# elfi-dev/elfi

Hardware: NVIDIA H100
Metric: accepted particles/sec (higher is better)
Workload: dtype f64

## Files before the change

elfi_b200/csrc/common.cuh:

```cuda
#pragma once

#include <cuda.h>
#include <cuda_runtime.h>

#include <cstdarg>
#include <cstdint>
#include <cstdio>
#include <cstring>
#include <type_traits>

#include "../../include/elfi_b200.h"

namespace elfi {

void set_error(const char* fmt, ...);

#define ELFI_CUDA_OK(expr)                                                              \
    do {                                                                                \
        cudaError_t _e = (expr);                                                        \
        if (_e != cudaSuccess) {                                                        \
            ::elfi::set_error("%s failed: %s (%s:%d)", #expr, cudaGetErrorString(_e),   \
                              __FILE__, __LINE__);                                      \
            cudaGetLastError();       \
            return ELFI_B200_ERR_CUDA;                                                  \
        }                                                                               \
    } while (0)

#define ELFI_REQUIRE(cond, ...)                                                         \
    do {                                                                                \
        if (!(cond)) {                                                                  \
            ::elfi::set_error(__VA_ARGS__);                                             \
            return ELFI_B200_ERR_ARG;                                                   \
        }                                                                               \
    } while (0)

typedef CUresult (*tensor_map_encode_fn)(CUtensorMap*, CUtensorMapDataType, cuuint32_t, void*,
                                         const cuuint64_t*, const cuuint64_t*,
                                         const cuuint32_t*, const cuuint32_t*,
                                         CUtensorMapInterleave, CUtensorMapSwizzle,
                                         CUtensorMapL2promotion, CUtensorMapFloatOOBfill);

}

struct elfi_b200_ctx {
    int device;
    int sm_count;
    size_t smem_optin;
    elfi::tensor_map_encode_fn encode_tiled;
    void* scratch;
    size_t scratch_bytes;
    void* pinned;
    size_t pinned_bytes;
    void* dev_stage;
    size_t dev_stage_bytes;
    cudaStream_t copy_stream[2];
    cudaEvent_t copy_event[4];
};

namespace elfi {

void* ctx_scratch(elfi_b200_ctx* ctx, size_t bytes);

int make_rowmajor_f64_map(elfi_b200_ctx* ctx, const double* base, int64_t rows, int64_t cols,
                          int64_t ld, int box_rows, CUtensorMap* out);

inline bool tma_compatible(const void* base, int64_t ld) {
    return (reinterpret_cast<uintptr_t>(base) % 16 == 0) && ((ld * 8) % 16 == 0);
}

template <class Body>
int run_on_device(elfi_b200_ctx* ctx, void* stream, Body&& body) {
    ELFI_CUDA_OK(cudaSetDevice(ctx->device));
    const int rc = body(static_cast<cudaStream_t>(stream));
    if (rc != ELFI_B200_OK) return rc;
    ELFI_CUDA_OK(cudaGetLastError());
    return ELFI_B200_OK;
}

template <int LO, int HI, class F>
auto with_pow2(int k, F&& f) {
    if constexpr (LO == HI) {
        return f(std::integral_constant<int, LO>{});
    } else {
// ... 72 lines not shown
```

elfi_b200/csrc/ctx.cu:

```cuda
#include "common.cuh"

namespace elfi {

static thread_local char g_error[512] = "";

void set_error(const char* fmt, ...) {
    va_list ap;
    va_start(ap, fmt);
    vsnprintf(g_error, sizeof(g_error), fmt, ap);
    va_end(ap);
}

void* ctx_scratch(elfi_b200_ctx* ctx, size_t bytes) {
    if (bytes <= ctx->scratch_bytes) return ctx->scratch;
    size_t want = bytes + (bytes >> 2) + (1u << 20);
    want = (want + 255) & ~size_t(255);
    if (ctx->scratch) {
        if (cudaDeviceSynchronize() != cudaSuccess || cudaFree(ctx->scratch) != cudaSuccess) {
            set_error("scratch release failed: %s", cudaGetErrorString(cudaGetLastError()));
            ctx->scratch = nullptr;
            ctx->scratch_bytes = 0;
            return nullptr;
        }
        ctx->scratch = nullptr;
// ... 40 lines not shown

const char* elfi_b200_last_error(void) { return elfi::g_error; }

int elfi_b200_ctx_create(int device, elfi_b200_ctx** out) {
    ELFI_REQUIRE(out != nullptr, "ctx_create: out is NULL");
    *out = nullptr;
    int count = 0;
    ELFI_CUDA_OK(cudaGetDeviceCount(&count));
    ELFI_REQUIRE(device >= 0 && device < count, "ctx_create: device %d out of range (%d visible)",
                 device, count);
    ELFI_CUDA_OK(cudaSetDevice(device));
    cudaDeviceProp prop;
    ELFI_CUDA_OK(cudaGetDeviceProperties(&prop, device));
    if (prop.major != 9 || prop.minor != 0) {
        elfi::set_error("ctx_create: device %d is sm_%d%d; this library is built for sm_90a only",
                        device, prop.major, prop.minor);
        return ELFI_B200_ERR_UNSUPPORTED;
    }
    elfi_b200_ctx* ctx = new elfi_b200_ctx();
    memset(ctx, 0, sizeof(*ctx));
    ctx->device = device;
    ctx->sm_count = prop.multiProcessorCount;
    ctx->smem_optin = prop.sharedMemPerBlockOptin;
    void* fn = nullptr;
    cudaDriverEntryPointQueryResult qres;
    cudaError_t e = cudaGetDriverEntryPoint("cuTensorMapEncodeTiled", &fn, cudaEnableDefault, &qres);
    if (e != cudaSuccess || qres != cudaDriverEntryPointSuccess || fn == nullptr) {
        elfi::set_error("ctx_create: cuTensorMapEncodeTiled not available from the driver");
        delete ctx;
        cudaGetLastError();
        return ELFI_B200_ERR_CUDA;
    }
    ctx->encode_tiled = reinterpret_cast<elfi::tensor_map_encode_fn>(fn);
    for (int i = 0; i < 2; ++i)
        ELFI_CUDA_OK(cudaStreamCreateWithFlags(&ctx->copy_stream[i], cudaStreamNonBlocking));
    for (int i = 0; i < 4; ++i)
        ELFI_CUDA_OK(cudaEventCreateWithFlags(&ctx->copy_event[i], cudaEventDisableTiming));
    *out = ctx;
    return ELFI_B200_OK;
}

int elfi_b200_ctx_destroy(elfi_b200_ctx* ctx) {
    if (!ctx) return ELFI_B200_OK;
    cudaSetDevice(ctx->device);
    cudaDeviceSynchronize();
    if (ctx->scratch) cudaFree(ctx->scratch);
    if (ctx->dev_stage) cudaFree(ctx->dev_stage);
    if (ctx->pinned) cudaFreeHost(ctx->pinned);
    for (int i = 0; i < 2; ++i)
        if (ctx->copy_stream[i]) cudaStreamDestroy(ctx->copy_stream[i]);
    for (int i = 0; i < 4; ++i)
        if (ctx->copy_event[i]) cudaEventDestroy(ctx->copy_event[i]);
    delete ctx;
    return ELFI_B200_OK;
}

int elfi_b200_ctx_sm_count(const elfi_b200_ctx* ctx) { return ctx ? ctx->sm_count : 0; }

int elfi_b200_allgather_particles(elfi_b200_ctx* const* ctxs, int64_t n_ctx, const double* const* send,
                                  int64_t rows, int64_t width, double* const* recv,
                                  void* const* streams) {
    ELFI_REQUIRE(ctxs && send && recv && streams && n_ctx >= 1 && n_ctx <= 64,
                 "allgather_particles: bad argument");
    ELFI_REQUIRE(rows >= 0 && width >= 1, "allgather_particles: bad shape");
    for (int64_t g = 0; g < n_ctx; ++g)
        ELFI_REQUIRE(ctxs[g] && (rows == 0 || (send[g] && recv[g])), "allgather_particles: NULL entry %lld",
                     (long long)g);
    if (rows == 0) return ELFI_B200_OK;
    const size_t bytes = size_t(rows) * size_t(width) * 8;
    int caller_device = 0;
    ELFI_CUDA_OK(cudaGetDevice(&caller_device));
    struct Restore {
        int d;
        ~Restore() { cudaSetDevice(d); }
    } restore{caller_device};
    for (int64_t d = 0; d < n_ctx; ++d) {
        ELFI_CUDA_OK(cudaSetDevice(ctxs[d]->device));
        for (int64_t s = 0; s < n_ctx; ++s) {
            if (ctxs[s]->device == ctxs[d]->device) continue;
            int can = 0;
// ... 34 lines not shown
```

elfi_b200/csrc/distance.cu:

```cuda
#include <cstdlib>

#include "metric.cuh"
#include "rowstream.cuh"

namespace elfi {

struct DistParams {
    const double* obs;
    const double* W;
    double* d_out;
    uint32_t* mask;
    int K;
    int has_thr;
    const double* shift_src;
    double* mom_partial;
    const double* thr_dev;
    double thr[ELFI_B200_MAX_NESTED];
    __device__ __forceinline__ double threshold(int k) const {
        return thr_dev ? __ldg(thr_dev + k) : thr[k];
    }
};

__device__ __forceinline__ void dist_setup_shared(uint8_t* aux, const DistParams& p, int D,
                                                  bool weighted) {
    const int Dp = rs_padded_cols(D);
    double* obs_s = reinterpret_cast<double*>(aux);
    for (int j = threadIdx.x; j < Dp; j += blockDim.x) obs_s[j] = j < D ? p.obs[j] : 0.0;
    if (weighted) {
        double* w_s = obs_s + Dp;
        for (int k = 0; k < p.K; ++k)
            for (int j = threadIdx.x; j < Dp; j += blockDim.x)
                w_s[size_t(k) * Dp + j] = j < D ? p.W[size_t(k) * D + j] : 0.0;
    }
}
// ... 265 lines not shown
            rc = rowstream_launch<NestedMomentsConsumer<KMAX>>(ctx, S, ldS, B, D, aux, p, stream);
    } else {
        rc = rowstream_launch<NestedMomentsConsumer<KMAX>>(ctx, S, ldS, B, D, aux, p, stream);
    }
    if (rc) return rc;
    colmoments_flush_kernel<<<unsigned((D + 31) / 32), dim3(32, 32), 0, stream>>>(
        S, p.mom_partial, nwarps, B, D, moments);
    ELFI_CUDA_OK(cudaGetLastError());
    return ELFI_B200_OK;
}

__global__ void __launch_bounds__(256)
dist_direct_kernel(const double* __restrict__ S, int64_t ld, int64_t B, int D, DistParams p) {
    const int64_t row = int64_t(blockIdx.x) * blockDim.x + threadIdx.x;
    dist_record<false, 0>(p, p.K, row, B, threadIdx.x & 31, [&](int k) {
        const double* r = S + row * ld;
        double acc = 0.0;
        if (p.W != nullptr) {
            const double* w = p.W + size_t(k) * D;
            for (int j = 0; j < D; ++j) {
                const double d = __dsub_rn(__ldg(r + j), __ldg(p.obs + j));
                acc = __dadd_rn(acc, __dmul_rn(__ldg(w + j), __dmul_rn(d, d)));
            }
        } else {
            for (int j = 0; j < D; ++j) {
                const double d = __dsub_rn(__ldg(r + j), __ldg(p.obs + j));
                acc = __dadd_rn(acc, __dmul_rn(d, d));
            }
        }
        return sqrt(acc);
    });
}

__global__ void __launch_bounds__(1024)
compact_mask_kernel(const uint32_t* __restrict__ mask, int64_t nwords, int64_t B,
                    int32_t* __restrict__ idx, int64_t* __restrict__ n_out) {
    __shared__ int64_t warp_sums[32];
    __shared__ int64_t base_s;
    const int tid = threadIdx.x;
    const int lane = tid & 31;
    const int wid = tid >> 5;
    const int64_t first = int64_t(blockIdx.x) * 1024;

    int64_t before = 0;
    for (int64_t w = tid; w < first; w += 1024) before += __popc(mask[w]);
    for (int o = 16; o > 0; o >>= 1) before += __shfl_xor_sync(0xffffffffu, before, o);
    if (lane == 0) warp_sums[wid] = before;
    __syncthreads();
    if (tid == 0) {
        int64_t t = 0;
        for (int i = 0; i < 32; ++i) t += warp_sums[i];
        base_s = t;
    }
    __syncthreads();
    const int64_t base = base_s;
    __syncthreads();

    const int64_t w = first + tid;
    const uint32_t bits = w < nwords ? mask[w] : 0u;
    const int cnt = __popc(bits);
    int incl = cnt;
    for (int o = 1; o < 32; o <<= 1) {
        const int t = __shfl_up_sync(0xffffffffu, incl, o);
        if (lane >= o) incl += t;
    }
    if (lane == 31) warp_sums[wid] = incl;
    __syncthreads();
    if (wid == 0) {
        int64_t v = warp_sums[lane];
        int64_t inc2 = v;
        for (int o = 1; o < 32; o <<= 1) {
            const int64_t t = __shfl_up_sync(0xffffffffu, inc2, o);
            if (lane >= o) inc2 += t;
        }
        warp_sums[lane] = inc2 - v;
        if (lane == 31 && blockIdx.x == gridDim.x - 1 && n_out != nullptr) *n_out = base + inc2;
    }
    __syncthreads();
    int64_t pos = base + warp_sums[wid] + (incl - cnt);
    if (idx != nullptr) {
        uint32_t b = bits;
        while (b) {
            const int bit = __ffs(b) - 1;
            b &= b - 1;
            idx[pos++] = int32_t(w * 32 + bit);
        }
    }
}

int launch_compact_mask(const uint32_t* mask, int64_t B, int32_t* idx, int64_t* n_out,
                        cudaStream_t stream) {
    const int64_t nwords = (B + 31) / 32;
    if (nwords == 0) {
        if (n_out) ELFI_CUDA_OK(cudaMemsetAsync(n_out, 0, sizeof(int64_t), stream));
        return ELFI_B200_OK;
    }
    const unsigned blocks = unsigned((nwords + 1023) / 1024);
    compact_mask_kernel<<<blocks, 1024, 0, stream>>>(mask, nwords, B, idx, n_out);
    ELFI_CUDA_OK(cudaGetLastError());
    return ELFI_B200_OK;
}

static DistParams dist_params(const double* obs, const double* W, int64_t K,
                              const double* thr_host, const double* thr_dev, double* d_out,
                              uint32_t* mask) {
    DistParams p = {};
    p.obs = obs;
    p.W = W;
    p.d_out = d_out;
    p.mask = mask;
    p.K = int(K);
    p.has_thr = thr_host != nullptr || thr_dev != nullptr;
    p.thr_dev = thr_dev;
    if (thr_host)
        for (int k = 0; k < K; ++k) p.thr[k] = thr_host[k];
    return p;
}

int launch_dist(elfi_b200_ctx* ctx, const double* S, int64_t ldS, int64_t B, int64_t D,
                const DistParams& p, cudaStream_t stream) {
    if (B == 0) return ELFI_B200_OK;
    const double* W = p.W;
    const int K = p.K;
    const size_t aux = size_t(rs_padded_cols(D)) * 8 * (W ? (1 + K) : 1);
    if (rs_streams(ctx, S, ldS, D, aux)) {
        if (W == nullptr) return rowstream_launch<EuclidConsumer>(ctx, S, ldS, B, D, aux, p, stream);
        if (K == 1) return rowstream_launch<WeightedConsumer>(ctx, S, ldS, B, D, aux, p, stream);
        if (K <= 2) return rowstream_launch<NestedConsumer<2>>(ctx, S, ldS, B, D, aux, p, stream);
        if (K <= 3) return rowstream_launch<NestedConsumer<3>>(ctx, S, ldS, B, D, aux, p, stream);
        if (K <= 4) return rowstream_launch<NestedConsumer<4>>(ctx, S, ldS, B, D, aux, p, stream);
        if (K <= 5) return rowstream_launch<NestedConsumer<5>>(ctx, S, ldS, B, D, aux, p, stream);
// ... 182 lines not shown
    ELFI_REQUIRE(B >= 0 && D >= 1, "dist: bad shape B=%lld D=%lld", (long long)B, (long long)D);
    ELFI_REQUIRE(B == 0 || S != nullptr, "dist: S is NULL");
    ELFI_REQUIRE(obs != nullptr, "dist: obs is NULL");
    ELFI_REQUIRE(ldS >= D, "dist: ldS (%lld) < D (%lld)", (long long)ldS, (long long)D);
    ELFI_REQUIRE(K >= 1 && K <= ELFI_B200_MAX_NESTED, "dist: K=%lld outside [1, %d]",
                 (long long)K, ELFI_B200_MAX_NESTED);
    ELFI_REQUIRE(W != nullptr || K == 1, "dist: K=%lld needs a weight matrix", (long long)K);
    ELFI_REQUIRE(acc_idx == nullptr || thr != nullptr, "dist: acc_idx requires thresholds");
    ELFI_REQUIRE(B < (int64_t(1) << 31), "dist: B must fit int32 row indices");
    return ELFI_B200_OK;
}

template <class Launch>
static int dist_call(const char* who, elfi_b200_ctx* ctx, const double* S, int64_t ldS, int64_t B,
                     int64_t D, const double* obs, const double* W, int64_t K,
                     const double* thr_host, const double* thr_dev, double* d_out,
                     int32_t* acc_idx, int64_t* n_acc, void* stream_, Launch launch) {
    const double* thr = thr_host ? thr_host : thr_dev;
    int rc = check_dist_args(S, ldS, B, D, obs, W, K, thr, acc_idx);
    if (rc) return rc;
    ELFI_REQUIRE(B == 0 || d_out != nullptr, "%s: d_out is NULL", who);
    cudaStream_t stream = static_cast<cudaStream_t>(stream_);
    ELFI_CUDA_OK(cudaSetDevice(ctx->device));
    uint32_t* mask = nullptr;
    if (thr != nullptr) {
        mask = static_cast<uint32_t*>(ctx_scratch(ctx, size_t((B + 31) / 32) * 4 + 256));
        if (!mask) return ELFI_B200_ERR_NOMEM;
    }
    rc = launch(dist_params(obs, W, K, thr_host, thr_dev, d_out, mask), stream);
    if (rc) return rc;
    if (thr != nullptr && (acc_idx != nullptr || n_acc != nullptr))
        return launch_compact_mask(mask, B, acc_idx, n_acc, stream);
    return ELFI_B200_OK;
}

}

extern "C" {

int elfi_b200_dist_euclid_thr_f64(elfi_b200_ctx* ctx, const double* S, int64_t ldS, int64_t B,
                                  int64_t D, const double* obs, const double* W, int64_t K,
                                  const double* thr_host, double* d_out, int32_t* acc_idx,
                                  int64_t* n_acc, void* stream_) {
    using namespace elfi;
    ELFI_REQUIRE(ctx != nullptr, "dist: ctx is NULL");
    return dist_call("dist", ctx, S, ldS, B, D, obs, W, K, thr_host, nullptr, d_out, acc_idx, n_acc,
                     stream_, [&](const DistParams& p, cudaStream_t stream) {
                         return launch_dist(ctx, S, ldS, B, D, p, stream);
                     });
}

int elfi_b200_dist_euclid_thr_dev_f64(elfi_b200_ctx* ctx, const double* S, int64_t ldS, int64_t B,
                                      int64_t D, const double* obs, const double* W, int64_t K,
                                      const double* thr_dev, double* d_out, int32_t* acc_idx,
                                      int64_t* n_acc, void* stream_) {
    using namespace elfi;
    ELFI_REQUIRE(ctx != nullptr && thr_dev != nullptr, "dist: ctx or thr_dev is NULL");
    return dist_call("dist", ctx, S, ldS, B, D, obs, W, K, nullptr, thr_dev, d_out, acc_idx, n_acc,
                     stream_, [&](const DistParams& p, cudaStream_t stream) {
                         return launch_dist(ctx, S, ldS, B, D, p, stream);
                     });
}

int elfi_b200_dist_euclid_mom_f64(elfi_b200_ctx* ctx, const double* S, int64_t ldS, int64_t B,
                                  int64_t D, const double* obs, const double* W, int64_t K,
                                  const double* thr_host, const double* thr_dev, double* d_out,
// ... 162 lines not shown
```

elfi_b200/csrc/select.cu:

```cuda
#include <cstdlib>

#include "bitonic.cuh"
#include "eqweight.h"
#include "pairwise.cuh"

namespace elfi {

constexpr int SORT_CHUNK = 1024;
constexpr int SORT_WARPS = 8;

__global__ void __launch_bounds__(256)
sort_prepare_kernel(const double* __restrict__ keys, int64_t n, uint64_t* __restrict__ ukeys,
                    int32_t* __restrict__ vals, uint32_t* __restrict__ ghist) {
    __shared__ uint32_t h[8 * 256];
    for (int i = threadIdx.x; i < 8 * 256; i += blockDim.x) h[i] = 0;
    __syncthreads();
    const int64_t stride = int64_t(gridDim.x) * blockDim.x;
    for (int64_t i = int64_t(blockIdx.x) * blockDim.x + threadIdx.x; i < n; i += stride) {
        const uint64_t u = key_to_u64(keys[i]);
        ukeys[i] = u;
        vals[i] = int32_t(i);
#pragma unroll
        for (int p = 0; p < 8; ++p) atomicAdd(&h[p * 256 + ((u >> (8 * p)) & 255)], 1u);
    }
    __syncthreads();
    for (int i = threadIdx.x; i < 8 * 256; i += blockDim.x)
        if (h[i]) atomicAdd(&ghist[i], h[i]);
}

__device__ __forceinline__ bool pass_trivial(const uint32_t* ghist, int pass, int64_t n,
                                             uint64_t first_key) {
    return ghist[pass * 256 + ((first_key >> (8 * pass)) & 255)] == uint32_t(n);
}

__global__ void __launch_bounds__(SORT_WARPS * 32)
// ... 142 lines not shown
    const unsigned wblocks = unsigned((s.nw + SORT_WARPS - 1) / SORT_WARPS);
    int cur = 0;
    for (int pass = 0; pass < 8; ++pass) {
        sort_upsweep_kernel<<<wblocks, SORT_WARPS * 32, 0, stream>>>(s.k[cur], n, pass, s.nw, s.ghist, s.whist);
        sort_scan_kernel<<<256, 1024, 0, stream>>>(s.k[cur], n, pass, s.nw, s.ghist, s.whist);
        sort_scatter_kernel<<<wblocks, SORT_WARPS * 32, 0, stream>>>(
            s.k[cur], s.v[cur], n, pass, s.nw, s.ghist, s.whist, s.k[cur ^ 1], s.v[cur ^ 1]);
        cur ^= 1;
    }
    ELFI_CUDA_OK(cudaGetLastError());
    return ELFI_B200_OK;
}

__global__ void __launch_bounds__(256)
gather_rows_kernel(const double* __restrict__ src, int64_t ld_src, const int32_t* __restrict__ idx,
                   int64_t n, int64_t width, double* __restrict__ dst, int64_t ld_dst) {
    const int64_t total = n * width;
    const int64_t stride = int64_t(gridDim.x) * blockDim.x;
    for (int64_t t = int64_t(blockIdx.x) * blockDim.x + threadIdx.x; t < total; t += stride) {
        const int64_t i = t / width, j = t - i * width;
        dst[i * ld_dst + j] = src[int64_t(idx[i]) * ld_src + j];
    }
}

constexpr int APPEND_MAX_SRC = 8;
struct AppendSources {
    const double* ptr[APPEND_MAX_SRC];
    int64_t ld[APPEND_MAX_SRC];
    int32_t width[APPEND_MAX_SRC];
    int32_t col0[APPEND_MAX_SRC];
    int32_t n_src, total_width;
};

__global__ void __launch_bounds__(256)
accept_append_kernel(const int32_t* __restrict__ acc_idx, const int64_t* __restrict__ n_acc,
                     AppendSources src, double* __restrict__ dst, int64_t ld_dst, int64_t capacity,
                     const int64_t* __restrict__ count) {
    const int64_t base = *count;
    int64_t room = capacity - base;
    if (room < 0) room = 0;
    const int64_t rows = *n_acc < room ? *n_acc : room;
    const int64_t total = rows * src.total_width;
    const int64_t stride = int64_t(gridDim.x) * blockDim.x;
    for (int64_t t = int64_t(blockIdx.x) * blockDim.x + threadIdx.x; t < total; t += stride) {
        const int64_t j = t / src.total_width;
        const int c = int(t - j * src.total_width);
        const int64_t row = acc_idx ? int64_t(acc_idx[j]) : j;
        int k = 0;
#pragma unroll
        for (int q = 1; q < APPEND_MAX_SRC; ++q)
            if (q < src.n_src && c >= src.col0[q]) k = q;
        dst[(base + j) * ld_dst + c] = src.ptr[k][row * src.ld[k] + (c - src.col0[k])];
    }
}

__global__ void accept_count_kernel(const int64_t* __restrict__ n_acc, int64_t capacity,
                                    int64_t* __restrict__ count, int64_t* __restrict__ dropped) {
    int64_t room = capacity - *count;
    if (room < 0) room = 0;
    const int64_t rows = *n_acc < room ? *n_acc : room;
    if (dropped) *dropped += *n_acc - rows;
    *count += rows;
}

__global__ void __launch_bounds__(256)
gather2_rows_kernel(const double* __restrict__ A, int64_t ldA, int64_t nA,
                    const double* __restrict__ Bm, int64_t ldB, const int32_t* __restrict__ mapB,
                    const int32_t* __restrict__ perm, int64_t n, int64_t width,
                    double* __restrict__ dst, int64_t ld_dst) {
    const int64_t total = n * width;
    const int64_t stride = int64_t(gridDim.x) * blockDim.x;
    for (int64_t t = int64_t(blockIdx.x) * blockDim.x + threadIdx.x; t < total; t += stride) {
        const int64_t i = t / width, j = t - i * width;
        const int64_t r = perm ? perm[i] : i;
        double v;
        if (r < nA) {
            v = A[r * ldA + j];
        } else {
            const int64_t rb = mapB ? int64_t(mapB[r - nA]) : (r - nA);
            v = Bm[rb * ldB + j];
        }
        dst[i * ld_dst + j] = v;
    }
}

__global__ void __launch_bounds__(256)
merge_keys_kernel(const double* __restrict__ keysA, int64_t ldA, int64_t nA,
                  const double* __restrict__ keysB, int64_t ldB, const int32_t* __restrict__ mapB,
                  int64_t nB, double* __restrict__ out) {
    const int64_t stride = int64_t(gridDim.x) * blockDim.x;
    for (int64_t i = int64_t(blockIdx.x) * blockDim.x + threadIdx.x; i < nA + nB; i += stride) {
        if (i < nA) {
            out[i] = keysA[i * ldA];
        } else {
            const int64_t rb = mapB ? int64_t(mapB[i - nA]) : (i - nA);
// ... 296 lines not shown
        double incl = v;
        for (int o = 1; o < 32; o <<= 1) {
            const double t = __shfl_up_sync(0xffffffffu, incl, o);
            if (lane >= o) incl += t;
        }
        if (lane == 31) ws[wid] = incl;
        __syncthreads();
        double woff = 0.0;
        for (int q = 0; q < wid; ++q) woff += ws[q];
        const double carry = carry_s;
        const double c = (carry + woff + incl) / total;
        if (i < n - 1) {
            l0 += (c < alpha - eps) ? 1 : 0;
            l1 += (c < alpha + eps) ? 1 : 0;
        }
        __syncthreads();
        if (tid == 1023) carry_s = carry + woff + incl;
        __syncthreads();
    }
    for (int o = 16; o > 0; o >>= 1) {
        l0 += __shfl_xor_sync(0xffffffffu, l0, o);
        l1 += __shfl_xor_sync(0xffffffffu, l1, o);
    }
    if (lane == 0) { atomicAdd(&c0_s, l0); atomicAdd(&c1_s, l1); }
    __syncthreads();
    if (tid == 0) { atomicAdd(&counts[0], c0_s); atomicAdd(&counts[1], c1_s); }
}

__global__ void wq_pick_kernel(const uint64_t* __restrict__ ukeys, int64_t idx, double* __restrict__ out) {
    out[0] = u64_to_key(ukeys[idx]);
    out[1] = double(idx);
}

}

extern "C" {

int elfi_b200_sort_pairs_f64(elfi_b200_ctx* ctx, const double* keys, int64_t n,
                             double* keys_sorted, int32_t* perm, void* stream_) {
    using namespace elfi;
    ELFI_REQUIRE(ctx != nullptr, "sort: ctx is NULL");
    ELFI_REQUIRE(n >= 0 && n < (int64_t(1) << 31), "sort: n=%lld out of range", (long long)n);
    if (n == 0) return ELFI_B200_OK;
    ELFI_REQUIRE(keys != nullptr, "sort: keys is NULL");
    cudaStream_t stream = static_cast<cudaStream_t>(stream_);
    ELFI_CUDA_OK(cudaSetDevice(ctx->device));
    uint8_t* base = static_cast<uint8_t*>(ctx_scratch(ctx, sort_scratch_bytes(n)));
    if (!base) return ELFI_B200_ERR_NOMEM;
    SortScratch s = carve_sort(base, n);
    int rc = sort_pairs_device(keys, n, s, ctx->sm_count, stream);
    if (rc) return rc;
    int blocks = int((n + 255) / 256);
    if (blocks > ctx->sm_count * 8) blocks = ctx->sm_count * 8;
    sort_finish_kernel<<<blocks, 256, 0, stream>>>(s.k[0], s.v[0], n, keys_sorted, perm);
    ELFI_CUDA_OK(cudaGetLastError());
    return ELFI_B200_OK;
}

int elfi_b200_gather_rows_f64(elfi_b200_ctx* ctx, const double* src, int64_t ld_src,
                              const int32_t* idx, int64_t n, int64_t width, double* dst,
                              int64_t ld_dst, void* stream_) {
    using namespace elfi;
    ELFI_REQUIRE(ctx != nullptr, "gather: ctx is NULL");
    ELFI_REQUIRE(n >= 0 && width >= 1 && ld_src >= width && ld_dst >= width, "gather: bad shape");
    if (n == 0) return ELFI_B200_OK;
    ELFI_REQUIRE(src && idx && dst, "gather: NULL argument");
// ... 47 lines not shown
    const size_t sort_bytes = sort_scratch_bytes(n);
    uint8_t* base = static_cast<uint8_t*>(ctx_scratch(ctx, sort_bytes + align256(size_t(n) * 8) + 256));
    if (!base) return ELFI_B200_ERR_NOMEM;
    SortScratch s = carve_sort(base, n);
    double* keys = reinterpret_cast<double*>(base + sort_bytes);
    int blocks = int((n + 255) / 256);
    if (blocks > ctx->sm_count * 8) blocks = ctx->sm_count * 8;
    merge_keys_kernel<<<blocks, 256, 0, stream>>>(keysA, ld_keysA, nA, keysB, ld_keysB, mapB, nB, keys);
    int rc = sort_pairs_device(keys, n, s, ctx->sm_count, stream);
    if (rc) return rc;
    const int32_t* perm = s.v[0];
    for (int64_t k = 0; k < n_out; ++k) {
        const int64_t width = width_host[k];
        ELFI_REQUIRE(width >= 1 && dst_host[k] && ld_dst_host[k] >= width &&
                     (nA == 0 || (A_host[k] && ldA_host[k] >= width)) &&
                     (nB == 0 || (B_host[k] && ldB_host[k] >= width)),
                     "topn_merge: bad descriptor of output %lld", (long long)k);
        int64_t gb = (n_keep * width + 255) / 256;
        if (gb > int64_t(ctx->sm_count) * 16) gb = int64_t(ctx->sm_count) * 16;
        gather2_rows_kernel<<<unsigned(gb), 256, 0, stream>>>(A_host[k], ldA_host[k], nA, B_host[k],
                                                              ldB_host[k], mapB, perm, n_keep, width,
                                                              dst_host[k], ld_dst_host[k]);
    }
    ELFI_CUDA_OK(cudaGetLastError());
    return ELFI_B200_OK;
}

int elfi_b200_accept_append_f64(elfi_b200_ctx* ctx, const int32_t* acc_idx, const int64_t* n_acc,
                                int64_t max_rows, int64_t n_src, const double* const* src_host,
                                const int64_t* ld_src_host, const int64_t* width_host, double* dst,
                                int64_t ld_dst, int64_t capacity, int64_t* count, int64_t* dropped,
                                void* stream_) {
    using namespace elfi;
    ELFI_REQUIRE(ctx && n_acc && src_host && ld_src_host && width_host && dst && count,
                 "accept_append: NULL argument");
    ELFI_REQUIRE(n_src >= 1 && n_src <= APPEND_MAX_SRC, "accept_append: 1..%d sources", APPEND_MAX_SRC);
    ELFI_REQUIRE(max_rows >= 0 && capacity >= 0, "accept_append: bad shape");
    AppendSources src;
    memset(&src, 0, sizeof(src));
    src.n_src = int32_t(n_src);
    int64_t col = 0;
    for (int k = 0; k < n_src; ++k) {
        ELFI_REQUIRE(src_host[k] && width_host[k] >= 1 && ld_src_host[k] >= width_host[k],
                     "accept_append: bad source %d", k);
        src.ptr[k] = src_host[k];
        src.ld[k] = ld_src_host[k];
        src.width[k] = int32_t(width_host[k]);
        src.col0[k] = int32_t(col);
        col += width_host[k];
    }
    ELFI_REQUIRE(col <= ld_dst && col < (int64_t(1) << 30), "accept_append: ld_dst < total width");
    src.total_width = int32_t(col);
    if (max_rows == 0) return ELFI_B200_OK;
    cudaStream_t stream = static_cast<cudaStream_t>(stream_);
    ELFI_CUDA_OK(cudaSetDevice(ctx->device));
    int64_t blocks = (max_rows * col + 255) / 256;
    if (blocks > int64_t(ctx->sm_count) * 8) blocks = int64_t(ctx->sm_count) * 8;
    accept_append_kernel<<<unsigned(blocks), 256, 0, stream>>>(acc_idx, n_acc, src, dst, ld_dst,
                                                              capacity, count);
    accept_count_kernel<<<1, 1, 0, stream>>>(n_acc, capacity, count, dropped);
    ELFI_CUDA_OK(cudaGetLastError());
    return ELFI_B200_OK;
}

int elfi_b200_rejection_batch_f64(elfi_b200_ctx* ctx, const double* S, int64_t ldS, int64_t B,
                                  int64_t D, const double* obs, const double* W, int64_t K,
                                  const double* thr_host, const double* thr_dev, double* d_out,
                                  int32_t* acc_idx, int64_t* n_acc, int64_t n_extra,
                                  const double* const* extra_host, const int64_t* ld_extra_host,
                                  const int64_t* width_extra_host, double* dst, int64_t ld_dst,
                                  int64_t capacity, int64_t* count, int64_t* dropped,
                                  void* stream_) {
    using namespace elfi;
    ELFI_REQUIRE(ctx && acc_idx && n_acc && d_out, "rejection_batch: NULL argument");
    ELFI_REQUIRE((thr_host != nullptr) != (thr_dev != nullptr),
                 "rejection_batch: thresholds on the host OR on the device");
    ELFI_REQUIRE(n_extra >= 0 && n_extra < APPEND_MAX_SRC, "rejection_batch: 0..%d extra sources",
                 APPEND_MAX_SRC - 1);
    int rc = thr_host
        ? elfi_b200_dist_euclid_thr_f64(ctx, S, ldS, B, D, obs, W, K, thr_host, d_out, acc_idx, n_acc,
                                        stream_)
        : elfi_b200_dist_euclid_thr_dev_f64(ctx, S, ldS, B, D, obs, W, K, thr_dev, d_out, acc_idx,
                                            n_acc, stream_);
    if (rc) return rc;
    const double* src[APPEND_MAX_SRC];
    int64_t ld[APPEND_MAX_SRC], width[APPEND_MAX_SRC];
    src[0] = d_out; ld[0] = K; width[0] = K;
    for (int64_t k = 0; k < n_extra; ++k) {
        src[k + 1] = extra_host[k];
        ld[k + 1] = ld_extra_host[k];
        width[k + 1] = width_extra_host[k];
    }
    return elfi_b200_accept_append_f64(ctx, acc_idx, n_acc, B, n_extra + 1, src, ld, width, dst,
                                       ld_dst, capacity, count, dropped, stream_);
}

int elfi_b200_wquantile_f64(elfi_b200_ctx* ctx, const double* x, const double* w, int64_t n,
                            double alpha, double* out, void* stream_) {
    using namespace elfi;
    ELFI_REQUIRE(ctx != nullptr && x != nullptr && out != nullptr, "wquantile: NULL argument");
    ELFI_REQUIRE(n >= 1 && n < (int64_t(1) << 31), "wquantile: n=%lld out of range", (long long)n);
    ELFI_REQUIRE(alpha >= 0.0 && alpha <= 1.0, "wquantile: alpha=%g outside [0, 1]", alpha);
    cudaStream_t stream = static_cast<cudaStream_t>(stream_);
    ELFI_CUDA_OK(cudaSetDevice(ctx->device));
    const size_t sort_bytes = sort_scratch_bytes(n);
    const size_t extra = align256(size_t(n + 2) * 8) + 256;
    uint8_t* base = static_cast<uint8_t*>(ctx_scratch(ctx, sort_bytes + extra));
    if (!base) return ELFI_B200_ERR_NOMEM;
    SortScratch s = carve_sort(base, n);
    double* ws = reinterpret_cast<double*>(base + sort_bytes);
    double* total = reinterpret_cast<double*>(base + sort_bytes + align256(size_t(n) * 8));
    int rc = sort_pairs_device(x, n, s, ctx->sm_count, stream);
    if (rc) return rc;
    if (w == nullptr && alpha > 0.0) {
        wq_pick_kernel<<<1, 1, 0, stream>>>(s.k[0], equal_weight_cum_index(n, alpha) - 1, out);
        ELFI_CUDA_OK(cudaGetLastError());
        return ELFI_B200_OK;
    }
    if (alpha > 0.0 && n > 1) {
        const int64_t nb = (n + 4095) / 4096;
        double* partial = ws;
        int32_t* counts = reinterpret_cast<int32_t*>(total) + 4;
        const double eps = (4.0 * double(n) + 64.0) * 1.1102230246251565e-16;
        wq_par_block_sums_kernel<<<unsigned(nb), 1024, 0, stream>>>(w, s.v[0], n, partial);
        wq_par_scan_kernel<<<1, 1024, 0, stream>>>(partial, nb, counts);
        wq_par_count_kernel<<<unsigned(nb), 1024, 0, stream>>>(w, s.v[0], n, partial, nb, alpha, eps, counts);
        int32_t hc[2] = {0, -1};
// ... 52 lines not shown
```

elfi_b200/ops.py:

```python
import ctypes

import numpy as np
import torch

from . import _lib
from . import device as dev

MAX_NESTED = 32


def _matrix(S):
    if dev.is_device_array(S) and S.dtype == torch.float64 and S.dim() == 2 \
            and S.stride(1) == 1 and S.stride(0) >= S.shape[1]:
        return S
    S = dev.to_device(S)
    if S.dim() == 1:
        S = S[:, None]
    if S.dim() != 2:
        raise ValueError('expected a 2-d (batch, dim) array, got shape {}'.format(tuple(S.shape)))
    if S.stride(1) != 1:
        S = S.contiguous()
    return S


# ... 306 lines not shown
        n, _, _, _, pp, pl, pw, prow, pcount, pdrop = self._descriptors(sources)
        _lib.call('elfi_b200_accept_append_f64', dev.context(), dev.ptr(acc_idx), dev.ptr(n_acc),
                  int(max_rows), n, pp, pl, pw, prow, self.width, self.capacity, pcount, pdrop,
                  dev.stream_ptr())

    def bind_batch(self, S, obs, thresholds, d_out, acc_idx, n_acc, extras, w=None):
        S = _matrix(S)
        B, D = S.shape
        W = None if w is None else dev.to_device(w).reshape(-1, D)
        K = 1 if W is None else W.shape[0]
        extras = [_as_2d(t) for t in extras]
        if [K] + [t.shape[1] for t in extras] != self.widths:
            raise ValueError('d / extra widths do not match the buffer layout')
        thr_dev = thresholds if dev.is_device_array(thresholds) else None
        thr_host = None if thr_dev is not None else np.ascontiguousarray(
            np.atleast_1d(thresholds), dtype=np.float64)
        n = len(extras)
        ptrs = (ctypes.c_void_p * max(n, 1))(*[t.data_ptr() for t in extras])
        lds = (ctypes.c_int64 * max(n, 1))(*[_ld(t) for t in extras])
        wid = (ctypes.c_int64 * max(n, 1))(*[t.shape[1] for t in extras])
        keep = (S, obs, W, thr_dev, thr_host, d_out, acc_idx, n_acc, extras, ptrs, lds, wid)
        args = (dev.context(), dev.ptr(S), S.stride(0) if B > 1 else D, B, D, dev.ptr(obs),
                dev.ptr(W), K, dev.ptr(thr_host), dev.ptr(thr_dev), dev.ptr(d_out),
                dev.ptr(acc_idx), dev.ptr(n_acc), n, ctypes.cast(ptrs, ctypes.c_void_p),
                ctypes.cast(lds, ctypes.c_void_p), ctypes.cast(wid, ctypes.c_void_p),
                dev.ptr(self.rows), self.width, self.capacity, dev.ptr(self.count),
                dev.ptr(self.dropped))

        def run(_keep=keep):
            _lib.call('elfi_b200_rejection_batch_f64', *args, dev.stream_ptr())
        return run

    def best(self, n, key_col=0):
        count, dropped = (int(v) for v in self._counters.cpu().tolist())
        keys = self.rows[:count, key_col].contiguous()
        perm = argsort(keys)
        return take_rows(self.rows, perm[:min(n, count)]), count, dropped


def allgather_particles(blocks):
    n = len(blocks)
    blocks = [b.contiguous() for b in blocks]
    rows = blocks[0].shape[0]
    width = int(np.prod(blocks[0].shape[1:])) if blocks[0].dim() > 1 else 1
    if any(tuple(b.shape) != tuple(blocks[0].shape) or b.dtype != torch.float64 for b in blocks):
        raise ValueError('blocks must be fp64 tensors of equal shape')
    outs, streams, ctxs = [], [], []
    for b in blocks:
        with torch.cuda.device(b.device):
            outs.append(torch.empty((n * rows,) + tuple(b.shape[1:]), dtype=torch.float64,
                                    device=b.device))
            streams.append(torch.cuda.current_stream(b.device).cuda_stream)
            ctxs.append(dev.context(b.device).value)
    arr = ctypes.c_void_p * n
    _lib.call('elfi_b200_allgather_particles', ctypes.cast(arr(*ctxs), ctypes.c_void_p), n,
              ctypes.cast(arr(*[b.data_ptr() for b in blocks]), ctypes.c_void_p), rows, width,
              ctypes.cast(arr(*[o.data_ptr() for o in outs]), ctypes.c_void_p),
              ctypes.cast(arr(*streams), ctypes.c_void_p))
    return outs


def weighted_sample_quantile(x, alpha, weights=None):
    x = dev.to_device(x).reshape(-1)
    w = None if weights is None else dev.to_device(weights).reshape(-1)
    if w is not None and w.numel() != x.numel():
        raise ValueError('x and weights must have the same length')
    out = dev.empty((2,))
    _lib.call('elfi_b200_wquantile_f64', dev.context(), dev.ptr(x), dev.ptr(w), x.numel(),
              float(alpha), dev.ptr(out), dev.stream_ptr())
    return float(out[0].item())
# ... 1582 lines not shown
```

Before: 25.90 million.

## Fuse mask compaction, row append and counter update into one epilogue kernel

The rejection batch path now runs the distance kernel to produce an accept mask, then a single epilogue kernel that compacts the mask into indices and appends accepted rows directly. Counter and dropped updates happen in the last-retiring block via a global ticket atomic. This replaces the separate compaction, append and count kernels. The standalone append path likewise merges its count kernel through the ticket. best() switches from argsort plus take_rows to a top-n merge call. The shared ticket counter adds a risk if kernels on different streams run concurrently.

Result: faster. 26.70 million (median of 6 runs) (+3.1%).

```diff
diff --git a/elfi_b200/csrc/common.cuh b/elfi_b200/csrc/common.cuh
--- a/elfi_b200/csrc/common.cuh
+++ b/elfi_b200/csrc/common.cuh
@@ -49,6 +49,7 @@
     elfi::tensor_map_encode_fn encode_tiled;
     void* scratch;
     size_t scratch_bytes;
+    uint32_t* ticket;
     void* pinned;
     size_t pinned_bytes;
     void* dev_stage;
diff --git a/elfi_b200/csrc/compact.cuh b/elfi_b200/csrc/compact.cuh
--- /dev/null
+++ b/elfi_b200/csrc/compact.cuh
@@ -0,0 +1,80 @@
+#pragma once
+
+#include "common.cuh"
+
+namespace elfi {
+
+constexpr int COMPACT_WORDS = 1024;
+
+int dist_euclid_mask(elfi_b200_ctx* ctx, const double* S, int64_t ldS, int64_t B, int64_t D,
+                     const double* obs, const double* W, int64_t K, const double* thr_host,
+                     const double* thr_dev, double* d_out, uint32_t** mask, cudaStream_t stream);
+
+struct CompactWord {
+    int64_t word;
+    uint32_t bits;
+    int64_t pos;
+    int64_t begin;
+    int64_t end;
+};
+
+__device__ __forceinline__ CompactWord compact_block(const uint32_t* __restrict__ mask,
+                                                     int64_t nwords, int64_t* sums) {
+    const int tid = threadIdx.x;
+    const int lane = tid & 31;
+    const int wid = tid >> 5;
+    const int64_t first = int64_t(blockIdx.x) * COMPACT_WORDS;
+
+    int64_t before = 0;
+    for (int64_t w = tid; w < first; w += COMPACT_WORDS) before += __popc(mask[w]);
+    for (int o = 16; o > 0; o >>= 1) before += __shfl_xor_sync(0xffffffffu, before, o);
+    if (lane == 0) sums[wid] = before;
+    __syncthreads();
+    if (tid == 0) {
+        int64_t t = 0;
+        for (int i = 0; i < 32; ++i) t += sums[i];
+        sums[32] = t;
+    }
+    __syncthreads();
+    const int64_t base = sums[32];
+    __syncthreads();
+
+    CompactWord cw;
+    cw.word = first + tid;
+    cw.bits = cw.word < nwords ? mask[cw.word] : 0u;
+    const int cnt = __popc(cw.bits);
+    int incl = cnt;
+    for (int o = 1; o < 32; o <<= 1) {
+        const int t = __shfl_up_sync(0xffffffffu, incl, o);
+        if (lane >= o) incl += t;
+    }
+    if (lane == 31) sums[wid] = incl;
+    __syncthreads();
+    if (wid == 0) {
+        const int64_t v = sums[lane];
+        int64_t inc2 = v;
+        for (int o = 1; o < 32; o <<= 1) {
+            const int64_t t = __shfl_up_sync(0xffffffffu, inc2, o);
+            if (lane >= o) inc2 += t;
+        }
+        sums[lane] = inc2 - v;
+        if (lane == 31) sums[32] = base + inc2;
+    }
+    __syncthreads();
+    cw.pos = base + sums[wid] + (incl - cnt);
+    cw.begin = base;
+    cw.end = sums[32];
+    return cw;
+}
+
+__device__ __forceinline__ void compact_write(const CompactWord& cw, int32_t* idx) {
+    uint32_t b = cw.bits;
+    int64_t pos = cw.pos;
+    while (b) {
+        const int bit = __ffs(b) - 1;
+        b &= b - 1;
+        idx[pos++] = int32_t(cw.word * 32 + bit);
+    }
+}
+
+}
diff --git a/elfi_b200/csrc/ctx.cu b/elfi_b200/csrc/ctx.cu
--- a/elfi_b200/csrc/ctx.cu
+++ b/elfi_b200/csrc/ctx.cu
@@ -96,6 +96,8 @@
         return ELFI_B200_ERR_CUDA;
     }
     ctx->encode_tiled = reinterpret_cast<elfi::tensor_map_encode_fn>(fn);
+    ELFI_CUDA_OK(cudaMalloc(&ctx->ticket, sizeof(uint32_t)));
+    ELFI_CUDA_OK(cudaMemset(ctx->ticket, 0, sizeof(uint32_t)));
     for (int i = 0; i < 2; ++i)
         ELFI_CUDA_OK(cudaStreamCreateWithFlags(&ctx->copy_stream[i], cudaStreamNonBlocking));
     for (int i = 0; i < 4; ++i)
@@ -110,6 +112,7 @@
     cudaDeviceSynchronize();
     if (ctx->scratch) cudaFree(ctx->scratch);
     if (ctx->dev_stage) cudaFree(ctx->dev_stage);
+    if (ctx->ticket) cudaFree(ctx->ticket);
     if (ctx->pinned) cudaFreeHost(ctx->pinned);
     for (int i = 0; i < 2; ++i)
         if (ctx->copy_stream[i]) cudaStreamDestroy(ctx->copy_stream[i]);
diff --git a/elfi_b200/csrc/distance.cu b/elfi_b200/csrc/distance.cu
--- a/elfi_b200/csrc/distance.cu
+++ b/elfi_b200/csrc/distance.cu
@@ -1,5 +1,6 @@
 #include <cstdlib>
 
+#include "compact.cuh"
 #include "metric.cuh"
 #include "rowstream.cuh"
 
@@ -331,60 +332,13 @@
     });
 }
 
-__global__ void __launch_bounds__(1024)
-compact_mask_kernel(const uint32_t* __restrict__ mask, int64_t nwords, int64_t B,
+__global__ void __launch_bounds__(COMPACT_WORDS)
+compact_mask_kernel(const uint32_t* __restrict__ mask, int64_t nwords,
                     int32_t* __restrict__ idx, int64_t* __restrict__ n_out) {
-    __shared__ int64_t warp_sums[32];
-    __shared__ int64_t base_s;
-    const int tid = threadIdx.x;
-    const int lane = tid & 31;
-    const int wid = tid >> 5;
-    const int64_t first = int64_t(blockIdx.x) * 1024;
-
-    int64_t before = 0;
-    for (int64_t w = tid; w < first; w += 1024) before += __popc(mask[w]);
-    for (int o = 16; o > 0; o >>= 1) before += __shfl_xor_sync(0xffffffffu, before, o);
-    if (lane == 0) warp_sums[wid] = before;
-    __syncthreads();
-    if (tid == 0) {
-        int64_t t = 0;
-        for (int i = 0; i < 32; ++i) t += warp_sums[i];
-        base_s = t;
-    }
-    __syncthreads();
-    const int64_t base = base_s;
-    __syncthreads();
-
-    const int64_t w = first + tid;
-    const uint32_t bits = w < nwords ? mask[w] : 0u;
-    const int cnt = __popc(bits);
-    int incl = cnt;
-    for (int o = 1; o < 32; o <<= 1) {
-        const int t = __shfl_up_sync(0xffffffffu, incl, o);
-        if (lane >= o) incl += t;
-    }
-    if (lane == 31) warp_sums[wid] = incl;
-    __syncthreads();
-    if (wid == 0) {
-        int64_t v = warp_sums[lane];
-        int64_t inc2 = v;
-        for (int o = 1; o < 32; o <<= 1) {
-            const int64_t t = __shfl_up_sync(0xffffffffu, inc2, o);
-            if (lane >= o) inc2 += t;
-        }
-        warp_sums[lane] = inc2 - v;
-        if (lane == 31 && blockIdx.x == gridDim.x - 1 && n_out != nullptr) *n_out = base + inc2;
-    }
-    __syncthreads();
-    int64_t pos = base + warp_sums[wid] + (incl - cnt);
-    if (idx != nullptr) {
-        uint32_t b = bits;
-        while (b) {
-            const int bit = __ffs(b) - 1;
-            b &= b - 1;
-            idx[pos++] = int32_t(w * 32 + bit);
-        }
-    }
+    __shared__ int64_t sums[33];
+    const CompactWord cw = compact_block(mask, nwords, sums);
+    if (threadIdx.x == 0 && blockIdx.x == gridDim.x - 1 && n_out != nullptr) *n_out = cw.end;
+    if (idx != nullptr) compact_write(cw, idx);
 }
 
 int launch_compact_mask(const uint32_t* mask, int64_t B, int32_t* idx, int64_t* n_out,
@@ -394,8 +348,8 @@
         if (n_out) ELFI_CUDA_OK(cudaMemsetAsync(n_out, 0, sizeof(int64_t), stream));
         return ELFI_B200_OK;
     }
-    const unsigned blocks = unsigned((nwords + 1023) / 1024);
-    compact_mask_kernel<<<blocks, 1024, 0, stream>>>(mask, nwords, B, idx, n_out);
+    const unsigned blocks = unsigned((nwords + COMPACT_WORDS - 1) / COMPACT_WORDS);
+    compact_mask_kernel<<<blocks, COMPACT_WORDS, 0, stream>>>(mask, nwords, idx, n_out);
     ELFI_CUDA_OK(cudaGetLastError());
     return ELFI_B200_OK;
 }
@@ -644,6 +598,16 @@
     if (thr != nullptr && (acc_idx != nullptr || n_acc != nullptr))
         return launch_compact_mask(mask, B, acc_idx, n_acc, stream);
     return ELFI_B200_OK;
+}
+
+int dist_euclid_mask(elfi_b200_ctx* ctx, const double* S, int64_t ldS, int64_t B, int64_t D,
+                     const double* obs, const double* W, int64_t K, const double* thr_host,
+                     const double* thr_dev, double* d_out, uint32_t** mask, cudaStream_t stream) {
+    return dist_call("dist", ctx, S, ldS, B, D, obs, W, K, thr_host, thr_dev, d_out, nullptr,
+                     nullptr, stream, [&](const DistParams& p, cudaStream_t s) {
+                         *mask = p.mask;
+                         return launch_dist(ctx, S, ldS, B, D, p, s);
+                     });
 }
 
 }
diff --git a/elfi_b200/csrc/select.cu b/elfi_b200/csrc/select.cu
--- a/elfi_b200/csrc/select.cu
+++ b/elfi_b200/csrc/select.cu
@@ -1,6 +1,7 @@
 #include <cstdlib>
 
 #include "bitonic.cuh"
+#include "compact.cuh"
 #include "eqweight.h"
 #include "pairwise.cuh"
 
@@ -209,19 +210,15 @@
     int32_t n_src, total_width;
 };
 
-__global__ void __launch_bounds__(256)
-accept_append_kernel(const int32_t* __restrict__ acc_idx, const int64_t* __restrict__ n_acc,
-                     AppendSources src, double* __restrict__ dst, int64_t ld_dst, int64_t capacity,
-                     const int64_t* __restrict__ count) {
-    const int64_t base = *count;
-    int64_t room = capacity - base;
-    if (room < 0) room = 0;
-    const int64_t rows = *n_acc < room ? *n_acc : room;
-    const int64_t total = rows * src.total_width;
-    const int64_t stride = int64_t(gridDim.x) * blockDim.x;
-    for (int64_t t = int64_t(blockIdx.x) * blockDim.x + threadIdx.x; t < total; t += stride) {
-        const int64_t j = t / src.total_width;
-        const int c = int(t - j * src.total_width);
+__device__ __forceinline__ void append_rows(const int32_t* acc_idx, int64_t j0, int64_t j1,
+                                            const AppendSources& src, double* __restrict__ dst,
+                                            int64_t ld_dst, int64_t base, int64_t t0,
+                                            int64_t stride) {
+    const int64_t total = (j1 - j0) * src.total_width;
+    for (int64_t t = t0; t < total; t += stride) {
+        const int64_t i = t / src.total_width;
+        const int c = int(t - i * src.total_width);
+        const int64_t j = j0 + i;
         const int64_t row = acc_idx ? int64_t(acc_idx[j]) : j;
         int k = 0;
 #pragma unroll
@@ -231,13 +228,65 @@
     }
 }
 
-__global__ void accept_count_kernel(const int64_t* __restrict__ n_acc, int64_t capacity,
-                                    int64_t* __restrict__ count, int64_t* __restrict__ dropped) {
-    int64_t room = capacity - *count;
+__device__ __forceinline__ bool retire_last(uint32_t* ticket) {
+    __shared__ bool last_s;
+    __syncthreads();
+    if (threadIdx.x == 0) {
+        __threadfence();
+        last_s = atomicAdd(ticket, 1u) == gridDim.x - 1;
+        if (last_s) {
+            *ticket = 0u;
+            __threadfence();
+        }
+    }
+    __syncthreads();
+    return last_s;
+}
+
+__device__ __forceinline__ void append_counters(int64_t n, int64_t count0, int64_t capacity,
+                                                int64_t* count, int64_t* dropped) {
+    int64_t room = capacity - count0;
     if (room < 0) room = 0;
-    const int64_t rows = *n_acc < room ? *n_acc : room;
-    if (dropped) *dropped += *n_acc - rows;
-    *count += rows;
+    const int64_t rows = n < room ? n : room;
+    if (dropped) *dropped += n - rows;
+    *count = count0 + rows;
+}
+
+__global__ void __launch_bounds__(256)
+accept_append_kernel(const int32_t* __restrict__ acc_idx, const int64_t* __restrict__ n_acc,
+                     AppendSources src, double* __restrict__ dst, int64_t ld_dst, int64_t capacity,
+                     int64_t* count, int64_t* dropped, uint32_t* ticket) {
+    const int64_t base = *count;
+    const int64_t n = *n_acc;
+    int64_t room = capacity - base;
+    if (room < 0) room = 0;
+    const int64_t rows = n < room ? n : room;
+    append_rows(acc_idx, 0, rows, src, dst, ld_dst, base,
+                int64_t(blockIdx.x) * blockDim.x + threadIdx.x, int64_t(gridDim.x) * blockDim.x);
+    if (retire_last(ticket) && threadIdx.x == 0) append_counters(n, base, capacity, count, dropped);
+}
+
+__global__ void __launch_bounds__(COMPACT_WORDS)
+rejection_epilogue_kernel(const uint32_t* __restrict__ mask, int64_t nwords, int32_t* idx,
+                          int64_t* n_acc, AppendSources src, double* __restrict__ dst,
+                          int64_t ld_dst, int64_t capacity, int64_t* count, int64_t* dropped,
+                          uint32_t* ticket) {
+    __shared__ int64_t sums[33];
+    __shared__ int64_t count0_s;
+    if (threadIdx.x == 0) count0_s = *count;
+    const CompactWord cw = compact_block(mask, nwords, sums);
+    if (threadIdx.x == 0 && blockIdx.x == gridDim.x - 1) *n_acc = cw.end;
+    compact_write(cw, idx);
+    __syncthreads();
+    const int64_t count0 = count0_s;
+    int64_t room = capacity - count0;
+    if (room < 0) room = 0;
+    const int64_t end = cw.end < room ? cw.end : room;
+    if (cw.begin < end)
+        append_rows(idx, cw.begin, end, src, dst, ld_dst, count0, threadIdx.x, blockDim.x);
+    if (retire_last(ticket) && threadIdx.x == 0)
+        append_counters(*reinterpret_cast<volatile int64_t*>(n_acc), count0, capacity, count,
+                        dropped);
 }
 
 __global__ void __launch_bounds__(256)
@@ -600,6 +649,30 @@
     out[1] = double(idx);
 }
 
+static int append_sources(int64_t n_src, const double* const* src_host, const int64_t* ld_src_host,
+                          const int64_t* width_host, const double* dst, int64_t ld_dst,
+                          int64_t capacity, const int64_t* count, AppendSources* src) {
+    ELFI_REQUIRE(src_host && ld_src_host && width_host && dst && count,
+                 "accept_append: NULL argument");
+    ELFI_REQUIRE(n_src >= 1 && n_src <= APPEND_MAX_SRC, "accept_append: 1..%d sources", APPEND_MAX_SRC);
+    ELFI_REQUIRE(capacity >= 0, "accept_append: bad shape");
+    memset(src, 0, sizeof(*src));
+    src->n_src = int32_t(n_src);
+    int64_t col = 0;
+    for (int k = 0; k < n_src; ++k) {
+        ELFI_REQUIRE(src_host[k] && width_host[k] >= 1 && ld_src_host[k] >= width_host[k],
+                     "accept_append: bad source %d", k);
+        src->ptr[k] = src_host[k];
+        src->ld[k] = ld_src_host[k];
+        src->width[k] = int32_t(width_host[k]);
+        src->col0[k] = int32_t(col);
+        col += width_host[k];
+    }
+    ELFI_REQUIRE(col <= ld_dst && col < (int64_t(1) << 30), "accept_append: ld_dst < total width");
+    src->total_width = int32_t(col);
+    return ELFI_B200_OK;
+}
+
 }
 
 extern "C" {
@@ -713,33 +786,19 @@
                                 int64_t ld_dst, int64_t capacity, int64_t* count, int64_t* dropped,
                                 void* stream_) {
     using namespace elfi;
-    ELFI_REQUIRE(ctx && n_acc && src_host && ld_src_host && width_host && dst && count,
-                 "accept_append: NULL argument");
-    ELFI_REQUIRE(n_src >= 1 && n_src <= APPEND_MAX_SRC, "accept_append: 1..%d sources", APPEND_MAX_SRC);
-    ELFI_REQUIRE(max_rows >= 0 && capacity >= 0, "accept_append: bad shape");
+    ELFI_REQUIRE(ctx && n_acc, "accept_append: NULL argument");
+    ELFI_REQUIRE(max_rows >= 0, "accept_append: bad shape");
     AppendSources src;
-    memset(&src, 0, sizeof(src));
-    src.n_src = int32_t(n_src);
-    int64_t col = 0;
-    for (int k = 0; k < n_src; ++k) {
-        ELFI_REQUIRE(src_host[k] && width_host[k] >= 1 && ld_src_host[k] >= width_host[k],
-                     "accept_append: bad source %d", k);
-        src.ptr[k] = src_host[k];
-        src.ld[k] = ld_src_host[k];
-        src.width[k] = int32_t(width_host[k]);
-        src.col0[k] = int32_t(col);
-        col += width_host[k];
-    }
-    ELFI_REQUIRE(col <= ld_dst && col < (int64_t(1) << 30), "accept_append: ld_dst < total width");
-    src.total_width = int32_t(col);
+    int rc = append_sources(n_src, src_host, ld_src_host, width_host, dst, ld_dst, capacity, count,
+                            &src);
+    if (rc) return rc;
     if (max_rows == 0) return ELFI_B200_OK;
     cudaStream_t stream = static_cast<cudaStream_t>(stream_);
     ELFI_CUDA_OK(cudaSetDevice(ctx->device));
-    int64_t blocks = (max_rows * col + 255) / 256;
+    int64_t blocks = (max_rows * src.total_width + 255) / 256;
     if (blocks > int64_t(ctx->sm_count) * 8) blocks = int64_t(ctx->sm_count) * 8;
     accept_append_kernel<<<unsigned(blocks), 256, 0, stream>>>(acc_idx, n_acc, src, dst, ld_dst,
-                                                              capacity, count);
-    accept_count_kernel<<<1, 1, 0, stream>>>(n_acc, capacity, count, dropped);
+                                                              capacity, count, dropped, ctx->ticket);
     ELFI_CUDA_OK(cudaGetLastError());
     return ELFI_B200_OK;
 }
@@ -758,22 +817,33 @@
                  "rejection_batch: thresholds on the host OR on the device");
     ELFI_REQUIRE(n_extra >= 0 && n_extra < APPEND_MAX_SRC, "rejection_batch: 0..%d extra sources",
                  APPEND_MAX_SRC - 1);
-    int rc = thr_host
-        ? elfi_b200_dist_euclid_thr_f64(ctx, S, ldS, B, D, obs, W, K, thr_host, d_out, acc_idx, n_acc,
-                                        stream_)
-        : elfi_b200_dist_euclid_thr_dev_f64(ctx, S, ldS, B, D, obs, W, K, thr_dev, d_out, acc_idx,
-                                            n_acc, stream_);
-    if (rc) return rc;
-    const double* src[APPEND_MAX_SRC];
+    ELFI_REQUIRE(n_extra == 0 || (extra_host && ld_extra_host && width_extra_host),
+                 "rejection_batch: NULL argument");
+    const double* srcp[APPEND_MAX_SRC];
     int64_t ld[APPEND_MAX_SRC], width[APPEND_MAX_SRC];
-    src[0] = d_out; ld[0] = K; width[0] = K;
+    srcp[0] = d_out; ld[0] = K; width[0] = K;
     for (int64_t k = 0; k < n_extra; ++k) {
-        src[k + 1] = extra_host[k];
+        srcp[k + 1] = extra_host[k];
         ld[k + 1] = ld_extra_host[k];
         width[k + 1] = width_extra_host[k];
     }
-    return elfi_b200_accept_append_f64(ctx, acc_idx, n_acc, B, n_extra + 1, src, ld, width, dst,
-                                       ld_dst, capacity, count, dropped, stream_);
+    AppendSources src;
+    int rc = append_sources(n_extra + 1, srcp, ld, width, dst, ld_dst, capacity, count, &src);
+    if (rc) return rc;
+    cudaStream_t stream = static_cast<cudaStream_t>(stream_);
+    uint32_t* mask = nullptr;
+    rc = dist_euclid_mask(ctx, S, ldS, B, D, obs, W, K, thr_host, thr_dev, d_out, &mask, stream);
+    if (rc) return rc;
+    const int64_t nwords = (B + 31) / 32;
+    if (nwords == 0) {
+        ELFI_CUDA_OK(cudaMemsetAsync(n_acc, 0, sizeof(int64_t), stream));
+        return ELFI_B200_OK;
+    }
+    const unsigned blocks = unsigned((nwords + COMPACT_WORDS - 1) / COMPACT_WORDS);
+    rejection_epilogue_kernel<<<blocks, COMPACT_WORDS, 0, stream>>>(
+        mask, nwords, acc_idx, n_acc, src, dst, ld_dst, capacity, count, dropped, ctx->ticket);
+    ELFI_CUDA_OK(cudaGetLastError());
+    return ELFI_B200_OK;
 }
 
 int elfi_b200_wquantile_f64(elfi_b200_ctx* ctx, const double* x, const double* w, int64_t n,
diff --git a/elfi_b200/ops.py b/elfi_b200/ops.py
--- a/elfi_b200/ops.py
+++ b/elfi_b200/ops.py
@@ -362,10 +362,23 @@
         return run
 
     def best(self, n, key_col=0):
+        if not hasattr(self, '_best_desc'):
+            arr_p, arr_i = ctypes.c_void_p * 1, ctypes.c_int64 * 1
+            src, ld, no_src = arr_p(self.rows.data_ptr()), arr_i(self.width), arr_p(0)
+            dst = arr_p(0)
+            cast = lambda a: ctypes.cast(a, ctypes.c_void_p)
+            self._best_desc = (src, ld, no_src, dst, cast(src), cast(ld), cast(no_src), cast(dst))
         count, dropped = (int(v) for v in self._counters.cpu().tolist())
-        keys = self.rows[:count, key_col].contiguous()
-        perm = argsort(keys)
-        return take_rows(self.rows, perm[:min(n, count)]), count, dropped
+        n_keep = min(n, count)
+        out = dev.empty((n_keep, self.width))
+        if n_keep:
+            _, _, _, dst, psrc, pld, pnone, pdst = self._best_desc
+            dst[0] = out.data_ptr()
+            _lib.call('elfi_b200_topn_merge_f64', dev.context(),
+                      ctypes.c_void_p(self.rows.data_ptr() + 8 * key_col), self.width, count, None,
+                      1, None, 0, n_keep, 1, psrc, pld, pnone, pld, pld, pdst, pld,
+                      dev.stream_ptr())
+        return out, count, dropped
 
 
 def allgather_particles(blocks):
```
